# petuum/autodist

Measured on AMD Instinct MI355X. Metric: images/sec ResNet-50 AllReduce, higher is better.
Workload: dtype bf16; 1 GPU; model=resnet50, global_batch=512, parallelism=dp1, image_size=224

## Files before the change

### autodist_amd/models/resnet.py

```python
import torch
import torch.nn as nn


def _make_bn(ch, fused, relu):
    if fused:
        from autodist_amd.ops.fused_bn import FusedBatchNorm2d
        return FusedBatchNorm2d(ch, relu=relu)
    return nn.BatchNorm2d(ch)


class Bottleneck(nn.Module):
    expansion = 4

    def __init__(self, in_ch, width, stride=1, downsample=None, fused=False):
        super().__init__()
        out_ch = width * self.expansion
        self.fused = fused
        self.conv1 = nn.Conv2d(in_ch, width, 1, bias=False)
        self.bn1 = _make_bn(width, fused, relu=True)
        self.conv2 = nn.Conv2d(width, width, 3, stride=stride, padding=1,
                               bias=False)
        self.bn2 = _make_bn(width, fused, relu=True)
        self.conv3 = nn.Conv2d(width, out_ch, 1, bias=False)
        self.bn3 = _make_bn(out_ch, fused, relu=True)
        self.relu = nn.ReLU(inplace=True)
        self.downsample = downsample

    def forward(self, x):
        if self.fused:
            out = self.bn1(self.conv1(x))
            out = self.bn2(self.conv2(out))
            z = self.conv3(out)
            if self.downsample is None:
                return self.bn3.forward_add(z, x)
            return self.bn3.forward_add_bn(z, self.downsample[0](x),
                                           self.downsample[1])
        identity = x
        out = self.relu(self.bn1(self.conv1(x)))
        out = self.relu(self.bn2(self.conv2(out)))
        out = self.bn3(self.conv3(out))
        if self.downsample is not None:
            identity = self.downsample(x)
        return self.relu(out + identity)


class BasicBlock(nn.Module):
    expansion = 1

    def __init__(self, in_ch, width, stride=1, downsample=None, fused=False):
        super().__init__()
        self.fused = fused
        self.conv1 = nn.Conv2d(in_ch, width, 3, stride=stride, padding=1,
                               bias=False)
        self.bn1 = _make_bn(width, fused, relu=True)
        self.conv2 = nn.Conv2d(width, width, 3, padding=1, bias=False)
        self.bn2 = _make_bn(width, fused, relu=True)
        self.relu = nn.ReLU(inplace=True)
        self.downsample = downsample

    def forward(self, x):
        if self.fused:
            out = self.bn1(self.conv1(x))
            z = self.conv2(out)
            if self.downsample is None:
                return self.bn2.forward_add(z, x)
            return self.bn2.forward_add_bn(z, self.downsample[0](x),
                                           self.downsample[1])
        identity = x
        out = self.relu(self.bn1(self.conv1(x)))
        out = self.bn2(self.conv2(out))
        if self.downsample is not None:
            identity = self.downsample(x)
        return self.relu(out + identity)


class ResNet(nn.Module):
    def __init__(self, block, layers, num_classes=1000, fused=False):
        super().__init__()
        self.in_ch = 64
        self.fused = fused
        self.conv1 = nn.Conv2d(3, 64, 7, stride=2, padding=3, bias=False)
        self.bn1 = _make_bn(64, fused, relu=True)
        self.relu = nn.ReLU(inplace=True)
        self.maxpool = nn.MaxPool2d(3, stride=2, padding=1)
        self.layer1 = self._make_layer(block, 64, layers[0])
        self.layer2 = self._make_layer(block, 128, layers[1], stride=2)
        self.layer3 = self._make_layer(block, 256, layers[2], stride=2)
        self.layer4 = self._make_layer(block, 512, layers[3], stride=2)
        self.avgpool = nn.AdaptiveAvgPool2d(1)
        self.fc = nn.Linear(512 * block.expansion, num_classes)
        from autodist_amd.ops.fused_bn import FusedBatchNorm2d
        for m in self.modules():
            if isinstance(m, nn.Conv2d):
                nn.init.kaiming_normal_(m.weight, mode="fan_out",
                                        nonlinearity="relu")
            elif isinstance(m, (nn.BatchNorm2d, FusedBatchNorm2d)):
                nn.init.ones_(m.weight)
                nn.init.zeros_(m.bias)

    def _make_layer(self, block, width, blocks, stride=1):
        downsample = None
        out_ch = width * block.expansion
        if stride != 1 or self.in_ch != out_ch:
            downsample = nn.Sequential(
                nn.Conv2d(self.in_ch, out_ch, 1, stride=stride, bias=False),
                _make_bn(out_ch, self.fused, relu=False))
        layers = [block(self.in_ch, width, stride, downsample,
                        fused=self.fused)]
        self.in_ch = out_ch
        for _ in range(1, blocks):
            layers.append(block(self.in_ch, width, fused=self.fused))
        return nn.Sequential(*layers)

    def forward(self, x):
        if self.fused:
            x = self.bn1.forward_pool(self.conv1(x))
        else:
            x = self.maxpool(self.relu(self.bn1(self.conv1(x))))
        x = self.layer4(self.layer3(self.layer2(self.layer1(x))))
        x = self.avgpool(x).flatten(1)
        return self.fc(x)


def resnet18(num_classes=1000, fused=False):
    return ResNet(BasicBlock, [2, 2, 2, 2], num_classes, fused=fused)


def resnet50(num_classes=1000, fused=False):
    return ResNet(Bottleneck, [3, 4, 6, 3], num_classes, fused=fused)


def resnet101(num_classes=1000, fused=False):
    return ResNet(Bottleneck, [3, 4, 23, 3], num_classes, fused=fused)
```

### autodist_amd/ops/csrc/bn_ops.hip

```cpp
#include "common.h"

#define BN_VEC 8
#define BN_RED_U 4
#define BN_FIN_U 8
#define BN_RELU_NONE 0
#define BN_RELU_Y 1
#define BN_RELU_MASK 2

__device__ __forceinline__ void load8(const __hip_bfloat16* p, float* v) {
  const __hip_bfloat162* p2 = reinterpret_cast<const __hip_bfloat162*>(p);
  float2 a = __bfloat1622float2(p2[0]);
  float2 b = __bfloat1622float2(p2[1]);
  float2 c = __bfloat1622float2(p2[2]);
  float2 d = __bfloat1622float2(p2[3]);
  v[0] = a.x; v[1] = a.y; v[2] = b.x; v[3] = b.y;
  v[4] = c.x; v[5] = c.y; v[6] = d.x; v[7] = d.y;
}
__device__ __forceinline__ void store8(__hip_bfloat16* p, const float* v) {
  __hip_bfloat162* p2 = reinterpret_cast<__hip_bfloat162*>(p);
  p2[0] = __float22bfloat162_rn({v[0], v[1]});
  p2[1] = __float22bfloat162_rn({v[2], v[3]});
  p2[2] = __float22bfloat162_rn({v[4], v[5]});
  p2[3] = __float22bfloat162_rn({v[6], v[7]});
}
// ... 390 lines not shown
  load8(dy + m * C + c0, dv);
  if (RELU == BN_RELU_Y) {
    float yv[BN_VEC];
    load8(y + m * C + c0, yv);
#pragma unroll
    for (int k = 0; k < BN_VEC; ++k) dv[k] = yv[k] > 0.f ? dv[k] : 0.f;
  }
  if (RELU == BN_RELU_MASK)
    apply_mask8(mask[m * (C / BN_VEC) + c0 / BN_VEC], dv);
}

template <typename T, int RELU>
__global__ void __launch_bounds__(BLOCK_THREADS)
__attribute__((amdgpu_waves_per_eu(RELU == BN_RELU_POOL ? 2 : 1)))
bn_bwd_reduce_kernel(const T* __restrict__ x, const T* __restrict__ dy,
                     const T* __restrict__ y,
                     const unsigned char* __restrict__ mask,
                     const float* __restrict__ save_mean,
                     const float* __restrict__ save_rstd,
                     float* __restrict__ partial_dz,
                     float* __restrict__ partial_dzxh, long M, int C,
                     BNPool pool) {
#pragma clang fp contract(off)
  int tx_count = min(C / BN_VEC, (int)blockDim.x);
  int tx = threadIdx.x % tx_count;
  int ty = threadIdx.x / tx_count;
  int rows_per_blk = blockDim.x / tx_count;
  int c0 = (blockIdx.y * tx_count + tx) * BN_VEC;
  if (c0 >= C) return;
  float mean[BN_VEC], rstd[BN_VEC];
  load8(save_mean + c0, mean);
  load8(save_rstd + c0, rstd);
  float s[BN_VEC] = {0}, t[BN_VEC] = {0};
  const long stride = (long)gridDim.x * rows_per_blk;
  long m = (long)blockIdx.x * rows_per_blk + ty;
  for (; m + (BN_RED_U - 1) * stride < M; m += BN_RED_U * stride) {
    Raw8<T> rx[BN_RED_U], rd[BN_RED_U], ry[BN_RED_U];
    unsigned rm[BN_RED_U];
    PoolTaps<T> rp[BN_RED_U];
#pragma unroll
    for (int u = 0; u < BN_RED_U; ++u) {
      const long mu = m + u * stride;
      rx[u] = load8raw(x + mu * C + c0);
      if (RELU == BN_RELU_POOL) {
        pool_issue(dy, pool, mu, C, c0, rp[u]);
        __builtin_amdgcn_sched_barrier(0);
      } else {
        rd[u] = load8raw(dy + mu * C + c0);
      }
      if (RELU == BN_RELU_Y) ry[u] = load8raw(y + mu * C + c0);
      if (RELU == BN_RELU_MASK) rm[u] = mask[mu * (C / BN_VEC) + c0 / BN_VEC];
    }
    __builtin_amdgcn_sched_barrier(0);
#pragma unroll
    for (int u = 0; u < BN_RED_U; ++u) {
      float xv[BN_VEC], dv[BN_VEC];
      unpack8(rx[u], xv);
      if (RELU == BN_RELU_POOL) pool_dz(rp[u], dv);
      else unpack8(rd[u], dv);
      if (RELU == BN_RELU_Y) {
        float yv[BN_VEC];
        unpack8(ry[u], yv);
#pragma unroll
        for (int k = 0; k < BN_VEC; ++k) dv[k] = yv[k] > 0.f ? dv[k] : 0.f;
      }
      if (RELU == BN_RELU_MASK) apply_mask8(rm[u], dv);
#pragma unroll
      for (int k = 0; k < BN_VEC; ++k) {
        s[k] += dv[k];
        t[k] = fmaf(dv[k] * (xv[k] - mean[k]), rstd[k], t[k]);
      }
      if (RELU == BN_RELU_POOL) __builtin_amdgcn_sched_barrier(0);
    }
  }
  for (; m < M; m += stride) {
    float xv[BN_VEC], dv[BN_VEC];
    load8(x + m * C + c0, xv);
    bn_load_dz<T, RELU>(dy, y, mask, pool, m, C, c0, dv);
#pragma unroll
    for (int k = 0; k < BN_VEC; ++k) {
      s[k] += dv[k];
      t[k] = fmaf(dv[k] * (xv[k] - mean[k]), rstd[k], t[k]);
    }
  }
  __shared__ float ls[BLOCK_THREADS * BN_VEC];
  __shared__ float lt[BLOCK_THREADS * BN_VEC];
#pragma unroll
  for (int k = 0; k < BN_VEC; ++k) {
    ls[threadIdx.x * BN_VEC + k] = s[k];
    lt[threadIdx.x * BN_VEC + k] = t[k];
  }
  __syncthreads();
  if (ty == 0) {
    for (int r = 1; r < rows_per_blk; ++r) {
      int o = (r * tx_count + tx) * BN_VEC;
#pragma unroll
      for (int k = 0; k < BN_VEC; ++k) { s[k] += ls[o + k]; t[k] += lt[o + k]; }
    }
    store8(partial_dz + (long)blockIdx.x * C + c0, s);
    store8(partial_dzxh + (long)blockIdx.x * C + c0, t);
  }
}

__global__ void bn_bwd_finalize_kernel(const float* __restrict__ partial_dz,
                                       const float* __restrict__ partial_dzxh,
                                       int grid_m,
                                       const float* __restrict__ weight,
                                       const float* __restrict__ save_rstd,
                                       float* __restrict__ k1,
                                       float* __restrict__ k2,
                                       float* __restrict__ k3,
                                       float* __restrict__ dweight,
                                       float* __restrict__ dbias, long M,
                                       int C) {
  int tx = threadIdx.x % FIN_CH;
  int ty = threadIdx.x / FIN_CH;
  int c = blockIdx.x * FIN_CH + tx;
  if (c >= C) return;
  float sdz = 0.f, sdzxh = 0.f;
  bn_fin_lane_sum(partial_dz, partial_dzxh, grid_m, ty, C, c, sdz, sdzxh);
  __shared__ float ls[FIN_LANES * FIN_CH], lq[FIN_LANES * FIN_CH];
  ls[ty * FIN_CH + tx] = sdz;
  lq[ty * FIN_CH + tx] = sdzxh;
  __syncthreads();
  if (ty != 0) return;
#pragma unroll
  for (int r = 1; r < FIN_LANES; ++r) {
    sdz += ls[r * FIN_CH + tx];
    sdzxh += lq[r * FIN_CH + tx];
  }
  k1[c] = weight[c] * save_rstd[c];
  k2[c] = sdz / (float)M;
  k3[c] = sdzxh / (float)M;
  dweight[c] = sdzxh;
  dbias[c] = sdz;
}

template <typename T, int RELU, bool ADD>
__global__ void bn_bwd_apply_kernel(const T* __restrict__ x,
                                    const T* __restrict__ dy,
                                    const T* __restrict__ y,
                                    const unsigned char* __restrict__ mask,
                                    const float* __restrict__ save_mean,
                                    const float* __restrict__ save_rstd,
                                    const float* __restrict__ k1,
                                    const float* __restrict__ k2,
                                    const float* __restrict__ k3,
                                    T* __restrict__ dx, T* __restrict__ dres,
                                    long M, int C, BNPool pool) {
  int tx_count = min(C / BN_VEC, (int)blockDim.x);
  int tx = threadIdx.x % tx_count;
  int ty = threadIdx.x / tx_count;
  int rows_per_blk = blockDim.x / tx_count;
  int c0 = (blockIdx.y * tx_count + tx) * BN_VEC;
  if (c0 >= C) return;
  float mean[BN_VEC], rstd[BN_VEC], a1[BN_VEC], a2[BN_VEC], a3[BN_VEC];
  load8(save_mean + c0, mean);
  load8(save_rstd + c0, rstd);
  load8(k1 + c0, a1);
  load8(k2 + c0, a2);
  load8(k3 + c0, a3);
  for (long m = (long)blockIdx.x * rows_per_blk + ty; m < M;
       m += (long)gridDim.x * rows_per_blk) {
    float xv[BN_VEC], dv[BN_VEC];
    load8(x + m * C + c0, xv);
    bn_load_dz<T, RELU>(dy, y, mask, pool, m, C, c0, dv);
// ... 11 lines not shown
```

### autodist_amd/ops/csrc/ext.hip

```cpp
#include <torch/extension.h>
#include <ATen/cuda/CUDAContext.h>

#include "multi_tensor.hip"
#include "bn_ops.hip"
#include "psgd_gemm.hip"
#include "mfma_probe.hip"
#include "attention.hip"
#include "attention_bwd.hip"
#include "ln_ops.hip"
#include "ce_ops.hip"

namespace {

inline hipStream_t cur_stream() {
  return at::cuda::getCurrentCUDAStream().stream();
}

struct BNGeom {
  long M;
  int C;
  int tx_count, rows_per_blk, grid_c;
};

BNGeom bn_geom(const torch::Tensor& x) {
// ... 289 lines not shown
  } else {
    yp = bn_ptr<const T>(yq);
  }
  float* wp = w5.data_ptr<float>();
  float* partial_dz = wp;
  float* partial_dzxh = wp + (long)BN_GM_MAX * g.C;
  float* k1 = wp + (long)(2 * BN_GM_MAX + 0) * g.C;
  float* k2 = wp + (long)(2 * BN_GM_MAX + 1) * g.C;
  float* k3 = wp + (long)(2 * BN_GM_MAX + 2) * g.C;
  auto dweight = torch::empty({g.C}, fopt);
  auto dbias = torch::empty({g.C}, fopt);
  auto dx = torch::empty_like(x);
  torch::Tensor dres;
  if (need_dres) dres = torch::empty_like(x);
  dim3 block(BLOCK_THREADS);
  int gm = bn_reduce_gm(g);
  dim3 grid_r(gm, g.grid_c);
  dim3 grid_a(bn_grid_m(g, 4096), g.grid_c);
  auto st = cur_stream();
  const float* sm = save_mean.data_ptr<float>();
  const float* sr = save_rstd.data_ptr<float>();

  hipLaunchKernelGGL((bn_bwd_reduce_kernel<T, RELU>), grid_r, block, 0, st,
                     bn_ptr<const T>(x), bn_ptr<const T>(dy), yp, mp, sm, sr,
                     partial_dz, partial_dzxh, g.M, g.C, BNPool{});
  hipLaunchKernelGGL(bn_bwd_finalize_kernel,
                     dim3((g.C + FIN_CH - 1) / FIN_CH),
                     dim3(FIN_CH * FIN_LANES), 0, st, partial_dz,
                     partial_dzxh, gm, weight.data_ptr<float>(), sr, k1, k2,
                     k3, dweight.data_ptr<float>(), dbias.data_ptr<float>(),
                     g.M, g.C);
  if (need_dres)
    hipLaunchKernelGGL((bn_bwd_apply_kernel<T, RELU, true>), grid_a, block, 0,
                       st, bn_ptr<const T>(x), bn_ptr<const T>(dy), yp, mp,
                       sm, sr, k1, k2, k3, bn_ptr<T>(dx), bn_ptr<T>(dres),
                       g.M, g.C, BNPool{});
  else
    hipLaunchKernelGGL((bn_bwd_apply_kernel<T, RELU, false>), grid_a, block,
                       0, st, bn_ptr<const T>(x), bn_ptr<const T>(dy), yp, mp,
                       sm, sr, k1, k2, k3, bn_ptr<T>(dx), (T*)nullptr, g.M,
                       g.C, BNPool{});
  std::vector<torch::Tensor> out = {dx, dweight, dbias};
  if (need_dres) out.push_back(dres);
  return out;
}

template <int RELU>
std::vector<torch::Tensor> bn_bwd_dispatch(
    const torch::Tensor& x, const torch::Tensor& dy, const torch::Tensor& yq,
    const torch::Tensor& save_mean, const torch::Tensor& save_rstd,
    const torch::Tensor& weight, bool need_dres,
    const c10::optional<torch::Tensor>& ws) {
  if (x.scalar_type() == torch::kBFloat16)
    return bn_bwd_impl<__hip_bfloat16, RELU>(x, dy, yq, save_mean, save_rstd,
                                             weight, need_dres, ws);
  TORCH_CHECK(x.scalar_type() == torch::kFloat32);
  return bn_bwd_impl<float, RELU>(x, dy, yq, save_mean, save_rstd, weight,
                                  need_dres, ws);
}

std::vector<torch::Tensor> bn_bwd(torch::Tensor x, torch::Tensor dy,
                                  torch::Tensor y, torch::Tensor save_mean,
                                  torch::Tensor save_rstd,
                                  torch::Tensor weight, bool relu,
                                  bool need_dres,
                                  c10::optional<torch::Tensor> ws) {
  if (relu)
    return bn_bwd_dispatch<BN_RELU_Y>(x, dy, y, save_mean, save_rstd, weight,
                                      need_dres, ws);
  return bn_bwd_dispatch<BN_RELU_NONE>(x, dy, y, save_mean, save_rstd, weight,
                                       need_dres, ws);
}

std::vector<torch::Tensor> bn_bwd_mask(torch::Tensor x, torch::Tensor dy,
                                       torch::Tensor mask,
                                       torch::Tensor save_mean,
                                       torch::Tensor save_rstd,
                                       torch::Tensor weight, bool relu,
                                       bool need_dres,
                                       c10::optional<torch::Tensor> ws) {
  TORCH_CHECK(relu, "the mask is the ReLU mask: relu must be set");
  return bn_bwd_dispatch<BN_RELU_MASK>(x, dy, mask, save_mean, save_rstd,
                                       weight, need_dres, ws);
}

template <typename T>
std::vector<torch::Tensor> bn_bwd_pool_impl(
    const torch::Tensor& x, const torch::Tensor& dy,
    const torch::Tensor& argmax, const torch::Tensor& save_mean,
    const torch::Tensor& save_rstd, const torch::Tensor& weight,
    const c10::optional<torch::Tensor>& ws) {
  auto g = bn_geom(x);
  BNPool p = bn_pool_geom(x, g);
  const long Mo = x.size(0) * (long)p.Ho * p.Wo;
  TORCH_CHECK(dy.dim() == 4 && dy.size(0) == x.size(0) && dy.size(1) == g.C &&
                  dy.size(2) == p.Ho && dy.size(3) == p.Wo &&
                  dy.scalar_type() == x.scalar_type() &&
                  dy.device() == x.device() &&
                  dy.is_contiguous(at::MemoryFormat::ChannelsLast),
              "dy must be the channels_last [N, C, Ho, Wo] gradient of the "
              "pooled y");
  TORCH_CHECK(argmax.scalar_type() == torch::kInt32 && argmax.is_contiguous() &&
                  argmax.dim() == 2 && argmax.size(0) == Mo &&
                  argmax.size(1) == g.C / BN_VEC &&
                  argmax.device() == x.device(),
              "argmax must be the [N*Ho*Wo, C/8] int32 tensor of "
              "bn_fwd_train_pool");
  p.amax = bn_ptr<const unsigned>(argmax);
  auto fopt = weight.options().dtype(torch::kFloat32);
  torch::Tensor w5 = ws.has_value() ? *ws
      : torch::empty({2 * BN_GM_MAX + 3, (long)g.C}, fopt);
  TORCH_CHECK(w5.size(0) >= 2 * BN_GM_MAX + 3 && w5.size(1) == g.C &&
              w5.is_contiguous());
  float* wp = w5.data_ptr<float>();
  float* partial_dz = wp;
  float* partial_dzxh = wp + (long)BN_GM_MAX * g.C;
  float* k1 = wp + (long)(2 * BN_GM_MAX + 0) * g.C;
  float* k2 = wp + (long)(2 * BN_GM_MAX + 1) * g.C;
  float* k3 = wp + (long)(2 * BN_GM_MAX + 2) * g.C;
  auto dweight = torch::empty({g.C}, fopt);
  auto dbias = torch::empty({g.C}, fopt);
  auto dx = torch::empty_like(x);
  dim3 block(BLOCK_THREADS);
  int gm = bn_reduce_gm(g);
  dim3 grid_r(gm, g.grid_c);
  dim3 grid_a(bn_grid_m(g, 4096), g.grid_c);
  auto st = cur_stream();
  const float* sm = save_mean.data_ptr<float>();
  const float* sr = save_rstd.data_ptr<float>();
  hipLaunchKernelGGL((bn_bwd_reduce_kernel<T, BN_RELU_POOL>), grid_r, block, 0,
                     st, bn_ptr<const T>(x), bn_ptr<const T>(dy),
                     (const T*)nullptr, (const unsigned char*)nullptr, sm, sr,
                     partial_dz, partial_dzxh, g.M, g.C, p);
  hipLaunchKernelGGL(bn_bwd_finalize_kernel,
                     dim3((g.C + FIN_CH - 1) / FIN_CH),
                     dim3(FIN_CH * FIN_LANES), 0, st, partial_dz,
                     partial_dzxh, gm, weight.data_ptr<float>(), sr, k1, k2,
                     k3, dweight.data_ptr<float>(), dbias.data_ptr<float>(),
                     g.M, g.C);
  hipLaunchKernelGGL((bn_bwd_apply_kernel<T, BN_RELU_POOL, false>), grid_a,
                     block, 0, st, bn_ptr<const T>(x), bn_ptr<const T>(dy),
                     (const T*)nullptr, (const unsigned char*)nullptr, sm, sr,
                     k1, k2, k3, bn_ptr<T>(dx), (T*)nullptr, g.M, g.C, p);
  return {dx, dweight, dbias};
}

std::vector<torch::Tensor> bn_bwd_pool(torch::Tensor x, torch::Tensor dy,
                                       torch::Tensor argmax,
                                       torch::Tensor save_mean,
                                       torch::Tensor save_rstd,
                                       torch::Tensor weight,
                                       c10::optional<torch::Tensor> ws) {
  if (x.scalar_type() == torch::kBFloat16)
    return bn_bwd_pool_impl<__hip_bfloat16>(x, dy, argmax, save_mean,
                                            save_rstd, weight, ws);
  TORCH_CHECK(x.scalar_type() == torch::kFloat32);
  return bn_bwd_pool_impl<float>(x, dy, argmax, save_mean, save_rstd, weight,
                                 ws);
}

void check_f32_flat(const torch::Tensor& t, const char* name) {
  TORCH_CHECK(t.is_cuda(), name, " must be on GPU");
  TORCH_CHECK(t.is_contiguous(), name, " must be contiguous");
  TORCH_CHECK(t.scalar_type() == torch::kFloat32, name, " must be fp32");
}

// ... 595 lines not shown
  long N = logits.size(0), H = logits.size(1);
  auto fopt = logits.options().dtype(torch::kFloat32);
  auto loss_rows = torch::empty({N}, fopt);
  auto m = torch::empty({N}, fopt);
  auto l2s = torch::empty({N}, fopt);
  hipLaunchKernelGGL(ce_fwd_kernel, dim3(N), dim3(256), 0, cur_stream(),
                     reinterpret_cast<__hip_bfloat16*>(logits.data_ptr()),
                     targets.data_ptr<long>(), loss_rows.data_ptr<float>(),
                     m.data_ptr<float>(), l2s.data_ptr<float>(), N, H);
  return {loss_rows, m, l2s};
}

torch::Tensor ce_bwd(torch::Tensor logits, torch::Tensor targets,
                     torch::Tensor m, torch::Tensor l2s,
                     torch::Tensor dloss_rows) {
  long N = logits.size(0), H = logits.size(1);
  auto dlogits = torch::empty_like(logits);
  hipLaunchKernelGGL(ce_bwd_kernel, dim3(N), dim3(256), 0, cur_stream(),
                     reinterpret_cast<__hip_bfloat16*>(logits.data_ptr()),
                     targets.data_ptr<long>(), m.data_ptr<float>(),
                     l2s.data_ptr<float>(),
                     dloss_rows.contiguous().data_ptr<float>(),
                     reinterpret_cast<__hip_bfloat16*>(dlogits.data_ptr()),
                     N, H);
  return dlogits;
}

torch::Tensor mfma_probe(torch::Tensor A, torch::Tensor B, long cand) {
  TORCH_CHECK(A.scalar_type() == torch::kBFloat16 && A.numel() == 16 * 32);
  TORCH_CHECK(B.scalar_type() == torch::kBFloat16 && B.numel() == 32 * 16);
  auto D = torch::zeros({16, 16}, A.options().dtype(torch::kFloat32));
  hipLaunchKernelGGL(mfma_probe_kernel, dim3(1), dim3(64), 0, cur_stream(),
                     reinterpret_cast<__hip_bfloat16*>(A.data_ptr()),
                     reinterpret_cast<__hip_bfloat16*>(B.data_ptr()),
                     D.data_ptr<float>(), (int)cand);
  return D;
}

void psgd_add_err_pad(torch::Tensor flat, torch::Tensor err,
                      torch::Tensor out) {
  long numel = flat.numel();
  long total = out.numel();
  hipLaunchKernelGGL(psgd_add_err_pad_kernel, dim3(grid_for(total, 1)),
                     dim3(BLOCK_THREADS), 0, cur_stream(),
                     flat.data_ptr<float>(), err.data_ptr<float>(),
                     out.data_ptr<float>(), numel, total);
}

}

PYBIND11_MODULE(TORCH_EXTENSION_NAME, m) {
  m.def("fused_sgd", &fused_sgd, "fused flat SGD update (gfx950)");
  m.def("fused_adam", &fused_adam, "fused flat Adam/AdamW update (gfx950)");
  m.def("fused_adagrad", &fused_adagrad,
        "fused flat Adagrad update (gfx950)");
  m.def("fused_sgd_wire", &fused_sgd_wire,
        "fused flat SGD update, bf16 wire gradient (gfx950)");
  m.def("fused_adam_wire", &fused_adam_wire,
        "fused flat Adam/AdamW update, bf16 wire gradient (gfx950)");
  m.def("fused_adagrad_wire", &fused_adagrad_wire,
        "fused flat Adagrad update, bf16 wire gradient (gfx950)");
  m.def("fused_rmsprop", &fused_rmsprop,
        "fused flat RMSprop update (gfx950, centered/momentum variants)");
  m.def("scale_cast_bf16", &scale_cast_bf16, "scale+cast fp32->bf16");
  m.def("cast_back_f32", &cast_back_f32, "cast bf16->fp32");
  m.def("ef_compress", &ef_compress, "fused error-feedback bf16 compress");
  m.def("segment_coalesce", &segment_coalesce,
        "dedup-sum row-sparse gradient");
  m.def("scatter_add_rows", &scatter_add_rows, "rowwise scatter-add");
  m.def("gather_rows", &gather_rows, "rowwise gather");
  m.def("sparse_apply_rows", &sparse_apply_rows,
        "fused row-wise SGD/Adagrad/Adam update of unique rows (gfx950)");
  m.def("bn_fwd_train", &bn_fwd_train,
        "fused NHWC batchnorm fwd (+add+relu), returns y/save_mean/save_rstd");
  m.def("bn_bwd", &bn_bwd,
        "fused NHWC batchnorm bwd (+relu-mask+dres), returns "
        "dx/dweight/dbias[/dres]");
  m.def("bn_fwd_train_mask", &bn_fwd_train_mask,
        "bn_fwd_train with relu that also returns the bit-packed ReLU mask "
        "[M, C/8] uint8");
  m.def("bn_bwd_mask", &bn_bwd_mask,
        "bn_bwd that takes the packed mask of bn_fwd_train_mask in place of "
        "y");
  m.def("bn_fwd_train_pool", &bn_fwd_train_pool,
        "bn + relu + 3x3/stride 2/pad 1 max-pool: (x, weight, bias, "
        "running_mean, running_var, eps, momentum, ws) -> (pooled y, "
        "save_mean, save_rstd, argmax words)");
  m.def("bn_bwd_pool", &bn_bwd_pool,
        "backward of bn_fwd_train_pool: (x, dy_pooled, argmax, save_mean, "
        "save_rstd, weight, ws) -> (dx, dweight, dbias)");
  m.def("bn_fwd_train_add_bn", &bn_fwd_train_add_bn,
        "relu(bn(z) + bn_d(zd)): (z, zd, then weight, bias, running_mean, "
        "running_var, eps, momentum, ws of each BN) -> (y, mask, save_mean, "
        "save_rstd, save_mean_d, save_rstd_d)");
  m.attr("BN_RED_U") = BN_RED_U;
  m.attr("BN_FIN_U") = BN_FIN_U;
  m.def("psgd_mq", &psgd_mq, "PowerSGD P = M @ Q (MFMA f32 16x16x4)");
  m.def("psgd_mtp", &psgd_mtp, "PowerSGD Qn = M^T @ P (MFMA f32 16x16x4)");
  m.def("psgd_decompress_ef", &psgd_decompress_ef,
        "fused hat = P Q^T * scale; err = M - hat; flat = hat");
  m.def("psgd_add_err_pad", &psgd_add_err_pad,
        "padded M = flat + err (zero tail)");
  m.def("mfma_probe", &mfma_probe,
        "diagnostic: v_mfma_f32_16x16x32_bf16 A/B layout probe");
  m.def("ce_fwd", &ce_fwd,
        "fused online-softmax cross-entropy fwd -> loss_rows, m, l2s");
  m.def("ce_bwd", &ce_bwd, "fused cross-entropy bwd -> dlogits (bf16)");
  m.def("col_sum", &col_sum, "bf16 [N,H] column sum -> fp32 [H]");
  m.def("ln_fwd", &ln_fwd,
        "fused bf16 LayerNorm(+residual) forward -> y, u, mean, rstd");
  m.def("ln_bwd", &ln_bwd, "fused bf16 LayerNorm backward -> dx, dgamma, "
        "dbeta");
  m.def("attn_dropmask", &attn_dropmask,
        "materialize the hash dropout keep-mask (testing)");
  m.def("attn_fwd", &attn_fwd,
        "fused MFMA attention forward (bf16, D=64; optional additive key "
        "mask + hash dropout) — 4-wave LDS-tiled",
        py::arg("q"), py::arg("k"), py::arg("v"), py::arg("scale"),
        py::arg("mask") = py::none(), py::arg("p_drop") = 0.0,
        py::arg("seed") = 0);
  m.def("attn_bwd", &attn_bwd,
        "fused MFMA attention backward (GPU-validated) -> dq, dk, dv",
        py::arg("q"), py::arg("k"), py::arg("v"), py::arg("o"),
        py::arg("dout"), py::arg("scale"), py::arg("mask") = py::none(),
        py::arg("p_drop") = 0.0, py::arg("seed") = 0);
}
```

### autodist_amd/ops/fused_bn.py

```python
from typing import Optional

import torch

from autodist_amd.ops import api as ops_api


SPLIT_PATH = False


class _FusedBNFunction(torch.autograd.Function):
    @staticmethod
    def forward(ctx, x, weight, bias, running_mean, running_var,
                momentum, eps, relu, residual, ws=None):
        use_hip = x.is_cuda and ops_api.has_gpu_ops()
        ctx.ws_bwd = ws[1] if ws is not None else None
        if use_hip and relu:
            y, save_mean, save_rstd, sign = ops_api.ext().bn_fwd_train_mask(
                x, weight, bias, running_mean, running_var, residual,
                eps, momentum, relu, ws[0] if ws is not None else None)
        elif use_hip:
            y, save_mean, save_rstd = ops_api.ext().bn_fwd_train(
                x, weight, bias, running_mean, running_var, residual,
                eps, momentum, relu, ws[0] if ws is not None else None)
            sign = y
        else:
            xf = x.float()
            m = xf.numel() // xf.size(1)
            with torch.no_grad():
                if m > 1:
                    y, save_mean, save_rstd = torch.native_batch_norm(
                        xf, weight, bias, running_mean, running_var, True,
                        momentum, eps)
                else:
                    y, save_mean, save_rstd = torch.native_batch_norm(
                        xf, weight, bias, None, None, True, momentum, eps)
                    running_mean.mul_(1 - momentum).add_(save_mean,
                                                         alpha=momentum)
                    running_var.mul_(1 - momentum)
                if residual is not None:
                    y = y + residual.float()
                if relu:
                    y = torch.relu(y)
                y = y.to(x.dtype)
            sign = y
        ctx.save_for_backward(x, sign, save_mean, save_rstd, weight)
        ctx.relu = relu
        ctx.has_res = residual is not None
        return y

    @staticmethod
    def backward(ctx, dy):
        x, sign, save_mean, save_rstd, weight = ctx.saved_tensors
        relu, has_res = ctx.relu, ctx.has_res
        use_hip = x.is_cuda and ops_api.has_gpu_ops()
        if use_hip:
            bwd = ops_api.ext().bn_bwd_mask if relu else ops_api.ext().bn_bwd
            out = bwd(x, dy.contiguous(
                memory_format=torch.channels_last), sign, save_mean, save_rstd,
                weight, relu, has_res, ctx.ws_bwd)
            dx, dweight, dbias = out[0], out[1], out[2]
            dres = out[3] if has_res else None
        else:
            dyf = dy.float()
            if relu:
                dyf = dyf * (sign > 0).float()
            dres = dyf.to(dy.dtype) if has_res else None
            dxf, dweight, dbias = torch.ops.aten.native_batch_norm_backward(
                dyf, x.float(), weight, None, None, save_mean, save_rstd,
                True, 0.0, [True, True, True])
            dx = dxf.to(x.dtype)
        return (dx, dweight, dbias, None, None, None, None, None, dres, None)


class _FusedBNPoolFunction(torch.autograd.Function):

    @staticmethod
    def forward(ctx, x, weight, bias, running_mean, running_var, momentum,
                eps, ws):
        y, save_mean, save_rstd, argmax = ops_api.ext().bn_fwd_train_pool(
            x, weight, bias, running_mean, running_var, eps, momentum,
            ws[0] if ws is not None else None)
        ctx.ws_bwd = ws[1] if ws is not None else None
        ctx.save_for_backward(x, argmax, save_mean, save_rstd, weight)
        return y

    @staticmethod
    def backward(ctx, dy):
        x, argmax, save_mean, save_rstd, weight = ctx.saved_tensors
        dx, dweight, dbias = ops_api.ext().bn_bwd_pool(
            x, dy.contiguous(memory_format=torch.channels_last), argmax,
            save_mean, save_rstd, weight, ctx.ws_bwd)
        return dx, dweight, dbias, None, None, None, None, None


class _FusedBNAddBNFunction(torch.autograd.Function):

    @staticmethod
    def forward(ctx, z, zd, weight, bias, running_mean, running_var, momentum,
                eps, ws, weight_d, bias_d, running_mean_d, running_var_d,
                momentum_d, eps_d, ws_d):
        y, mask, sm, sr, sm_d, sr_d = ops_api.ext().bn_fwd_train_add_bn(
            z, zd, weight, bias, running_mean, running_var, eps, momentum,
            ws[0] if ws is not None else None,
            weight_d, bias_d, running_mean_d, running_var_d, eps_d,
            momentum_d, ws_d[0] if ws_d is not None else None)
        ctx.ws_bwd = ws[1] if ws is not None else None
        ctx.ws_bwd_d = ws_d[1] if ws_d is not None else None
        ctx.save_for_backward(z, zd, mask, sm, sr, sm_d, sr_d, weight,
                              weight_d)
        return y

    @staticmethod
    def backward(ctx, dy):
        z, zd, mask, sm, sr, sm_d, sr_d, weight, weight_d = ctx.saved_tensors
        dy = dy.contiguous(memory_format=torch.channels_last)
        bwd = ops_api.ext().bn_bwd_mask
        dz, dw, db = bwd(z, dy, mask, sm, sr, weight, True, False, ctx.ws_bwd)
        dzd, dw_d, db_d = bwd(zd, dy, mask, sm_d, sr_d, weight_d, True, False,
                              ctx.ws_bwd_d)
        return (dz, dzd, dw, db, None, None, None, None, None,
                dw_d, db_d, None, None, None, None, None)


def fused_bn_train(x, weight, bias, running_mean, running_var,
                   momentum=0.1, eps=1e-5, relu=False,
                   residual: Optional[torch.Tensor] = None, ws=None):
    return _FusedBNFunction.apply(x, weight, bias, running_mean, running_var,
                                  momentum, eps, relu, residual, ws)


class FusedBatchNorm2d(torch.nn.Module):

    def __init__(self, num_features, eps=1e-5, momentum=0.1, relu=False):
        super().__init__()
        self.num_features = num_features
        self.eps = eps
        self.momentum = momentum
        self.relu = relu
        self.weight = torch.nn.Parameter(torch.ones(num_features))
        self.bias = torch.nn.Parameter(torch.zeros(num_features))
        self.register_buffer("running_mean", torch.zeros(num_features))
        self.register_buffer("running_var", torch.ones(num_features))
        self.register_buffer("num_batches_tracked",
                             torch.tensor(0, dtype=torch.long))
        self._ws = None

    def _check(self, x):
        if x.is_cuda and not x.is_contiguous(memory_format=torch.channels_last):
            x = x.contiguous(memory_format=torch.channels_last)
        return x

    def _workspace(self, x):
        if not x.is_cuda:
            return None
        if self._ws is None or self._ws[0].device != x.device:
            self._ws = (
                torch.empty(2 * 512 + 4, self.num_features, device=x.device),
                torch.empty(2 * 512 + 3, self.num_features, device=x.device))
        return self._ws

    def forward(self, x, residual: Optional[torch.Tensor] = None):
        x = self._check(x)
        if residual is not None:
            residual = self._check(residual)
        if self.training:
            self.num_batches_tracked += 1
            return fused_bn_train(x, self.weight, self.bias,
                                  self.running_mean, self.running_var,
                                  self.momentum, self.eps, self.relu, residual,
                                  ws=self._workspace(x))
        scale = self.weight * (self.running_var + self.eps).rsqrt()
        shift = self.bias - self.running_mean * scale
        y = x * scale[None, :, None, None].to(x.dtype) + \
            shift[None, :, None, None].to(x.dtype)
        if residual is not None:
            y = y + residual
        return torch.relu(y) if self.relu else y

    def forward_add(self, x, residual):
        return self.forward(x, residual)

    def _fused_kernels(self, x):
        return (self.training and x.is_cuda and ops_api.has_gpu_ops()
                and not SPLIT_PATH)

    def forward_pool(self, x):
        assert self.relu, "forward_pool is bn -> relu -> max-pool"
        if not self._fused_kernels(x):
            return torch.nn.functional.max_pool2d(self.forward(x), 3, 2, 1)
        x = self._check(x)
        self.num_batches_tracked += 1
        return _FusedBNPoolFunction.apply(
            x, self.weight, self.bias, self.running_mean, self.running_var,
            self.momentum, self.eps, self._workspace(x))

    def forward_add_bn(self, z, zd, other_bn):
        if not (self._fused_kernels(z) and self.relu
                and isinstance(other_bn, FusedBatchNorm2d)
                and other_bn.training and not other_bn.relu):
            return self.forward_add(z, other_bn(zd))
        z, zd = self._check(z), other_bn._check(zd)
        self.num_batches_tracked += 1
        other_bn.num_batches_tracked += 1
        return _FusedBNAddBNFunction.apply(
            z, zd, self.weight, self.bias, self.running_mean,
            self.running_var, self.momentum, self.eps, self._workspace(z),
            other_bn.weight, other_bn.bias, other_bn.running_mean,
            other_bn.running_var, other_bn.momentum, other_bn.eps,
            other_bn._workspace(zd))

    def extra_repr(self):
        return f"{self.num_features}, relu={self.relu}"
```

Before: 9638 images/sec.

## Fuse residual gradient add into BN backward reduce via paired block outputs

```diff
diff --git a/autodist_amd/models/resnet.py b/autodist_amd/models/resnet.py
--- a/autodist_amd/models/resnet.py
+++ b/autodist_amd/models/resnet.py
@@ -26,15 +26,19 @@
         self.relu = nn.ReLU(inplace=True)
         self.downsample = downsample
 
+    def forward_pair(self, xs):
+        x_main, x_res = xs
+        out = self.bn1(self.conv1(x_main))
+        out = self.bn2(self.conv2(out))
+        z = self.conv3(out)
+        if self.downsample is None:
+            return self.bn3.forward_add_pair(z, x_res)
+        return self.bn3.forward_add_bn_pair(z, self.downsample[0](x_res),
+                                            self.downsample[1])
+
     def forward(self, x):
         if self.fused:
-            out = self.bn1(self.conv1(x))
-            out = self.bn2(self.conv2(out))
-            z = self.conv3(out)
-            if self.downsample is None:
-                return self.bn3.forward_add(z, x)
-            return self.bn3.forward_add_bn(z, self.downsample[0](x),
-                                           self.downsample[1])
+            return self.forward_pair((x, x))[0]
         identity = x
         out = self.relu(self.bn1(self.conv1(x)))
         out = self.relu(self.bn2(self.conv2(out)))
@@ -58,14 +62,18 @@
         self.relu = nn.ReLU(inplace=True)
         self.downsample = downsample
 
+    def forward_pair(self, xs):
+        x_main, x_res = xs
+        out = self.bn1(self.conv1(x_main))
+        z = self.conv2(out)
+        if self.downsample is None:
+            return self.bn2.forward_add_pair(z, x_res)
+        return self.bn2.forward_add_bn_pair(z, self.downsample[0](x_res),
+                                            self.downsample[1])
+
     def forward(self, x):
         if self.fused:
-            out = self.bn1(self.conv1(x))
-            z = self.conv2(out)
-            if self.downsample is None:
-                return self.bn2.forward_add(z, x)
-            return self.bn2.forward_add_bn(z, self.downsample[0](x),
-                                           self.downsample[1])
+            return self.forward_pair((x, x))[0]
         identity = x
         out = self.relu(self.bn1(self.conv1(x)))
         out = self.bn2(self.conv2(out))
@@ -115,9 +123,14 @@
     def forward(self, x):
         if self.fused:
             x = self.bn1.forward_pool(self.conv1(x))
+            xs = (x, x)
+            for layer in (self.layer1, self.layer2, self.layer3, self.layer4):
+                for block in layer:
+                    xs = block.forward_pair(xs)
+            x = xs[0]
         else:
             x = self.maxpool(self.relu(self.bn1(self.conv1(x))))
-        x = self.layer4(self.layer3(self.layer2(self.layer1(x))))
+            x = self.layer4(self.layer3(self.layer2(self.layer1(x))))
         x = self.avgpool(x).flatten(1)
         return self.fc(x)
 
diff --git a/autodist_amd/ops/csrc/bn_ops.hip b/autodist_amd/ops/csrc/bn_ops.hip
--- a/autodist_amd/ops/csrc/bn_ops.hip
+++ b/autodist_amd/ops/csrc/bn_ops.hip
@@ -496,6 +496,102 @@
       s[k] += dv[k];
       t[k] = fmaf(dv[k] * (xv[k] - mean[k]), rstd[k], t[k]);
     }
+  }
+  __shared__ float ls[BLOCK_THREADS * BN_VEC];
+  __shared__ float lt[BLOCK_THREADS * BN_VEC];
+#pragma unroll
+  for (int k = 0; k < BN_VEC; ++k) {
+    ls[threadIdx.x * BN_VEC + k] = s[k];
+    lt[threadIdx.x * BN_VEC + k] = t[k];
+  }
+  __syncthreads();
+  if (ty == 0) {
+    for (int r = 1; r < rows_per_blk; ++r) {
+      int o = (r * tx_count + tx) * BN_VEC;
+#pragma unroll
+      for (int k = 0; k < BN_VEC; ++k) { s[k] += ls[o + k]; t[k] += lt[o + k]; }
+    }
+    store8(partial_dz + (long)blockIdx.x * C + c0, s);
+    store8(partial_dzxh + (long)blockIdx.x * C + c0, t);
+  }
+}
+
+#ifndef BN_JOIN_U
+#define BN_JOIN_U 4
+#endif
+template <typename T>
+__device__ __forceinline__ void bn_join_dz8(const float* av, const float* bv,
+                                            unsigned bits, float* dv) {
+#pragma clang fp contract(off)
+#pragma unroll
+  for (int k = 0; k < BN_VEC; ++k)
+    dv[k] = (bits >> k) & 1u ? round_to(av[k] + bv[k], (const T*)nullptr)
+                             : 0.f;
+}
+
+template <typename T>
+__global__ void __launch_bounds__(BLOCK_THREADS)
+__attribute__((amdgpu_waves_per_eu(1)))
+bn_bwd_reduce_join_kernel(const T* __restrict__ x, const T* __restrict__ dy_a,
+                          const T* __restrict__ dy_b,
+                          const unsigned char* __restrict__ mask,
+                          const float* __restrict__ save_mean,
+                          const float* __restrict__ save_rstd,
+                          float* __restrict__ partial_dz,
+                          float* __restrict__ partial_dzxh,
+                          T* __restrict__ dz, long M, int C) {
+#pragma clang fp contract(off)
+  int tx_count = min(C / BN_VEC, (int)blockDim.x);
+  int tx = threadIdx.x % tx_count;
+  int ty = threadIdx.x / tx_count;
+  int rows_per_blk = blockDim.x / tx_count;
+  int c0 = (blockIdx.y * tx_count + tx) * BN_VEC;
+  if (c0 >= C) return;
+  float mean[BN_VEC], rstd[BN_VEC];
+  load8(save_mean + c0, mean);
+  load8(save_rstd + c0, rstd);
+  float s[BN_VEC] = {0}, t[BN_VEC] = {0};
+  const long stride = (long)gridDim.x * rows_per_blk;
+  long m = (long)blockIdx.x * rows_per_blk + ty;
+  for (; m + (BN_JOIN_U - 1) * stride < M; m += BN_JOIN_U * stride) {
+    Raw8<T> rx[BN_JOIN_U], ra[BN_JOIN_U], rb[BN_JOIN_U];
+    unsigned rm[BN_JOIN_U];
+#pragma unroll
+    for (int u = 0; u < BN_JOIN_U; ++u) {
+      const long mu = m + u * stride;
+      rx[u] = load8raw(x + mu * C + c0);
+      ra[u] = load8raw(dy_a + mu * C + c0);
+      rb[u] = load8raw(dy_b + mu * C + c0);
+      rm[u] = mask[mu * (C / BN_VEC) + c0 / BN_VEC];
+    }
+    __builtin_amdgcn_sched_barrier(0);
+#pragma unroll
+    for (int u = 0; u < BN_JOIN_U; ++u) {
+      float xv[BN_VEC], av[BN_VEC], bv[BN_VEC], dv[BN_VEC];
+      unpack8(rx[u], xv);
+      unpack8(ra[u], av);
+      unpack8(rb[u], bv);
+      bn_join_dz8<T>(av, bv, rm[u], dv);
+#pragma unroll
+      for (int k = 0; k < BN_VEC; ++k) {
+        s[k] += dv[k];
+        t[k] = fmaf(dv[k] * (xv[k] - mean[k]), rstd[k], t[k]);
+      }
+      store8(dz + (m + u * stride) * C + c0, dv);
+    }
+  }
+  for (; m < M; m += stride) {
+    float xv[BN_VEC], av[BN_VEC], bv[BN_VEC], dv[BN_VEC];
+    load8(x + m * C + c0, xv);
+    load8(dy_a + m * C + c0, av);
+    load8(dy_b + m * C + c0, bv);
+    bn_join_dz8<T>(av, bv, mask[m * (C / BN_VEC) + c0 / BN_VEC], dv);
+#pragma unroll
+    for (int k = 0; k < BN_VEC; ++k) {
+      s[k] += dv[k];
+      t[k] = fmaf(dv[k] * (xv[k] - mean[k]), rstd[k], t[k]);
+    }
+    store8(dz + m * C + c0, dv);
   }
   __shared__ float ls[BLOCK_THREADS * BN_VEC];
   __shared__ float lt[BLOCK_THREADS * BN_VEC];
diff --git a/autodist_amd/ops/csrc/ext.hip b/autodist_amd/ops/csrc/ext.hip
--- a/autodist_amd/ops/csrc/ext.hip
+++ b/autodist_amd/ops/csrc/ext.hip
@@ -395,6 +395,79 @@
   TORCH_CHECK(relu, "the mask is the ReLU mask: relu must be set");
   return bn_bwd_dispatch<BN_RELU_MASK>(x, dy, mask, save_mean, save_rstd,
                                        weight, need_dres, ws);
+}
+
+template <typename T>
+std::vector<torch::Tensor> bn_bwd_mask_join_impl(
+    const torch::Tensor& x, const torch::Tensor& dy_a,
+    const torch::Tensor& dy_b, const torch::Tensor& mask,
+    const torch::Tensor& save_mean, const torch::Tensor& save_rstd,
+    const torch::Tensor& weight, const c10::optional<torch::Tensor>& ws) {
+  auto g = bn_geom(x);
+  for (const torch::Tensor* d : {&dy_a, &dy_b})
+    TORCH_CHECK(d->sizes() == x.sizes() &&
+                    d->scalar_type() == x.scalar_type() &&
+                    d->device() == x.device() &&
+                    d->is_contiguous(at::MemoryFormat::ChannelsLast),
+                "bn_bwd_mask_join: dy_a and dy_b must match x in shape, "
+                "dtype, device and channels_last layout");
+  auto fopt = weight.options().dtype(torch::kFloat32);
+  torch::Tensor w5 = ws.has_value() ? *ws
+      : torch::empty({2 * BN_GM_MAX + 3, (long)g.C}, fopt);
+  TORCH_CHECK(w5.size(0) >= 2 * BN_GM_MAX + 3 && w5.size(1) == g.C &&
+              w5.is_contiguous());
+  TORCH_CHECK(mask.scalar_type() == torch::kUInt8 && mask.is_contiguous() &&
+                  mask.dim() == 2 && mask.size(0) == g.M &&
+                  mask.size(1) == g.C / BN_VEC && mask.device() == x.device(),
+              "mask must be the [M, C/8] uint8 tensor of bn_fwd_train_mask");
+  const unsigned char* mp = mask.data_ptr<unsigned char>();
+  float* wp = w5.data_ptr<float>();
+  float* partial_dz = wp;
+  float* partial_dzxh = wp + (long)BN_GM_MAX * g.C;
+  float* k1 = wp + (long)(2 * BN_GM_MAX + 0) * g.C;
+  float* k2 = wp + (long)(2 * BN_GM_MAX + 1) * g.C;
+  float* k3 = wp + (long)(2 * BN_GM_MAX + 2) * g.C;
+  auto dweight = torch::empty({g.C}, fopt);
+  auto dbias = torch::empty({g.C}, fopt);
+  auto dx = torch::empty_like(x);
+  auto dz = torch::empty_like(x);
+  dim3 block(BLOCK_THREADS);
+  int gm = bn_reduce_gm(g);
+  dim3 grid_r(gm, g.grid_c);
+  dim3 grid_a(bn_grid_m(g, 4096), g.grid_c);
+  auto st = cur_stream();
+  const float* sm = save_mean.data_ptr<float>();
+  const float* sr = save_rstd.data_ptr<float>();
+
+  hipLaunchKernelGGL((bn_bwd_reduce_join_kernel<T>), grid_r, block, 0, st,
+                     bn_ptr<const T>(x), bn_ptr<const T>(dy_a),
+                     bn_ptr<const T>(dy_b), mp, sm, sr, partial_dz,
+                     partial_dzxh, bn_ptr<T>(dz), g.M, g.C);
+  hipLaunchKernelGGL(bn_bwd_finalize_kernel,
+                     dim3((g.C + FIN_CH - 1) / FIN_CH),
+                     dim3(FIN_CH * FIN_LANES), 0, st, partial_dz,
+                     partial_dzxh, gm, weight.data_ptr<float>(), sr, k1, k2,
+                     k3, dweight.data_ptr<float>(), dbias.data_ptr<float>(),
+                     g.M, g.C);
+  hipLaunchKernelGGL((bn_bwd_apply_kernel<T, BN_RELU_NONE, false>), grid_a,
+                     block, 0, st, bn_ptr<const T>(x), bn_ptr<const T>(dz),
+                     (const T*)nullptr, (const unsigned char*)nullptr, sm, sr,
+                     k1, k2, k3, bn_ptr<T>(dx), (T*)nullptr, g.M, g.C,
+                     BNPool{});
+  return {dx, dweight, dbias, dz};
+}
+
+std::vector<torch::Tensor> bn_bwd_mask_join(
+    torch::Tensor x, torch::Tensor dy_a, torch::Tensor dy_b,
+    torch::Tensor mask, torch::Tensor save_mean, torch::Tensor save_rstd,
+    torch::Tensor weight, c10::optional<torch::Tensor> ws) {
+  if (x.scalar_type() == torch::kBFloat16)
+    return bn_bwd_mask_join_impl<__hip_bfloat16>(x, dy_a, dy_b, mask,
+                                                 save_mean, save_rstd, weight,
+                                                 ws);
+  TORCH_CHECK(x.scalar_type() == torch::kFloat32);
+  return bn_bwd_mask_join_impl<float>(x, dy_a, dy_b, mask, save_mean,
+                                      save_rstd, weight, ws);
 }
 
 template <typename T>
@@ -1156,6 +1229,10 @@
   m.def("bn_bwd_mask", &bn_bwd_mask,
         "bn_bwd that takes the packed mask of bn_fwd_train_mask in place of "
         "y");
+  m.def("bn_bwd_mask_join", &bn_bwd_mask_join,
+        "bn_bwd_mask for dy = dy_a + dy_b, the add done in the reduce: (x, "
+        "dy_a, dy_b, mask, save_mean, save_rstd, weight, ws) -> (dx, "
+        "dweight, dbias, dz); dz is the masked sum, the split path's dres");
   m.def("bn_fwd_train_pool", &bn_fwd_train_pool,
         "bn + relu + 3x3/stride 2/pad 1 max-pool: (x, weight, bias, "
         "running_mean, running_var, eps, momentum, ws) -> (pooled y, "
@@ -1169,6 +1246,7 @@
         "save_rstd, save_mean_d, save_rstd_d)");
   m.attr("BN_RED_U") = BN_RED_U;
   m.attr("BN_FIN_U") = BN_FIN_U;
+  m.attr("BN_JOIN_U") = BN_JOIN_U;
   m.def("psgd_mq", &psgd_mq, "PowerSGD P = M @ Q (MFMA f32 16x16x4)");
   m.def("psgd_mtp", &psgd_mtp, "PowerSGD Qn = M^T @ P (MFMA f32 16x16x4)");
   m.def("psgd_decompress_ef", &psgd_decompress_ef,
diff --git a/autodist_amd/ops/fused_bn.py b/autodist_amd/ops/fused_bn.py
--- a/autodist_amd/ops/fused_bn.py
+++ b/autodist_amd/ops/fused_bn.py
@@ -8,11 +8,22 @@
 SPLIT_PATH = False
 
 
+def _two_handles(ctx, y):
+    ctx.set_materialize_grads(False)
+    return y, y.view_as(y)
+
+
+def _nhwc_grad(g):
+    return None if g is None else g.contiguous(
+        memory_format=torch.channels_last)
+
+
 class _FusedBNFunction(torch.autograd.Function):
     @staticmethod
     def forward(ctx, x, weight, bias, running_mean, running_var,
-                momentum, eps, relu, residual, ws=None):
+                momentum, eps, relu, residual, ws=None, pair=False):
         use_hip = x.is_cuda and ops_api.has_gpu_ops()
+        assert not pair or (use_hip and relu and residual is not None)
         ctx.ws_bwd = ws[1] if ws is not None else None
         if use_hip and relu:
             y, save_mean, save_rstd, sign = ops_api.ext().bn_fwd_train_mask(
@@ -46,14 +57,22 @@
         ctx.save_for_backward(x, sign, save_mean, save_rstd, weight)
         ctx.relu = relu
         ctx.has_res = residual is not None
-        return y
-
-    @staticmethod
-    def backward(ctx, dy):
+        return _two_handles(ctx, y) if pair else y
+
+    @staticmethod
+    def backward(ctx, dy, dy_b=None):
         x, sign, save_mean, save_rstd, weight = ctx.saved_tensors
         relu, has_res = ctx.relu, ctx.has_res
         use_hip = x.is_cuda and ops_api.has_gpu_ops()
-        if use_hip:
+        if dy is None:
+            dy, dy_b = dy_b, None
+            if dy is None:
+                return (None,) * 11
+        if dy_b is not None:
+            dx, dweight, dbias, dres = ops_api.ext().bn_bwd_mask_join(
+                x, _nhwc_grad(dy), _nhwc_grad(dy_b), sign, save_mean,
+                save_rstd, weight, ctx.ws_bwd)
+        elif use_hip:
             bwd = ops_api.ext().bn_bwd_mask if relu else ops_api.ext().bn_bwd
             out = bwd(x, dy.contiguous(
                 memory_format=torch.channels_last), sign, save_mean, save_rstd,
@@ -69,7 +88,8 @@
                 dyf, x.float(), weight, None, None, save_mean, save_rstd,
                 True, 0.0, [True, True, True])
             dx = dxf.to(x.dtype)
-        return (dx, dweight, dbias, None, None, None, None, None, dres, None)
+        return (dx, dweight, dbias, None, None, None, None, None, dres, None,
+                None)
 
 
 class _FusedBNPoolFunction(torch.autograd.Function):
@@ -98,7 +118,7 @@
     @staticmethod
     def forward(ctx, z, zd, weight, bias, running_mean, running_var, momentum,
                 eps, ws, weight_d, bias_d, running_mean_d, running_var_d,
-                momentum_d, eps_d, ws_d):
+                momentum_d, eps_d, ws_d, pair=False):
         y, mask, sm, sr, sm_d, sr_d = ops_api.ext().bn_fwd_train_add_bn(
             z, zd, weight, bias, running_mean, running_var, eps, momentum,
             ws[0] if ws is not None else None,
@@ -108,25 +128,38 @@
         ctx.ws_bwd_d = ws_d[1] if ws_d is not None else None
         ctx.save_for_backward(z, zd, mask, sm, sr, sm_d, sr_d, weight,
                               weight_d)
-        return y
-
-    @staticmethod
-    def backward(ctx, dy):
+        return _two_handles(ctx, y) if pair else y
+
+    @staticmethod
+    def backward(ctx, dy, dy_b=None):
         z, zd, mask, sm, sr, sm_d, sr_d, weight, weight_d = ctx.saved_tensors
-        dy = dy.contiguous(memory_format=torch.channels_last)
-        bwd = ops_api.ext().bn_bwd_mask
-        dz, dw, db = bwd(z, dy, mask, sm, sr, weight, True, False, ctx.ws_bwd)
-        dzd, dw_d, db_d = bwd(zd, dy, mask, sm_d, sr_d, weight_d, True, False,
-                              ctx.ws_bwd_d)
+        if dy is None:
+            dy, dy_b = dy_b, None
+            if dy is None:
+                return (None,) * 17
+        dy = _nhwc_grad(dy)
+        if dy_b is not None:
+            dz, dw, db, dym = ops_api.ext().bn_bwd_mask_join(
+                z, dy, _nhwc_grad(dy_b), mask, sm, sr, weight, ctx.ws_bwd)
+            dzd, dw_d, db_d = ops_api.ext().bn_bwd(
+                zd, dym, dym, sm_d, sr_d, weight_d, False, False,
+                ctx.ws_bwd_d)
+        else:
+            bwd = ops_api.ext().bn_bwd_mask
+            dz, dw, db = bwd(z, dy, mask, sm, sr, weight, True, False,
+                             ctx.ws_bwd)
+            dzd, dw_d, db_d = bwd(zd, dy, mask, sm_d, sr_d, weight_d, True,
+                                  False, ctx.ws_bwd_d)
         return (dz, dzd, dw, db, None, None, None, None, None,
-                dw_d, db_d, None, None, None, None, None)
+                dw_d, db_d, None, None, None, None, None, None)
 
 
 def fused_bn_train(x, weight, bias, running_mean, running_var,
                    momentum=0.1, eps=1e-5, relu=False,
-                   residual: Optional[torch.Tensor] = None, ws=None):
+                   residual: Optional[torch.Tensor] = None, ws=None,
+                   pair=False):
     return _FusedBNFunction.apply(x, weight, bias, running_mean, running_var,
-                                  momentum, eps, relu, residual, ws)
+                                  momentum, eps, relu, residual, ws, pair)
 
 
 class FusedBatchNorm2d(torch.nn.Module):
@@ -184,6 +217,17 @@
         return (self.training and x.is_cuda and ops_api.has_gpu_ops()
                 and not SPLIT_PATH)
 
+    def forward_add_pair(self, x, residual):
+        if not (self._fused_kernels(x) and self.relu):
+            y = self.forward_add(x, residual)
+            return y, y
+        self.num_batches_tracked += 1
+        return fused_bn_train(self._check(x), self.weight, self.bias,
+                              self.running_mean, self.running_var,
+                              self.momentum, self.eps, True,
+                              self._check(residual), ws=self._workspace(x),
+                              pair=True)
+
     def forward_pool(self, x):
         assert self.relu, "forward_pool is bn -> relu -> max-pool"
         if not self._fused_kernels(x):
@@ -194,11 +238,15 @@
             x, self.weight, self.bias, self.running_mean, self.running_var,
             self.momentum, self.eps, self._workspace(x))
 
-    def forward_add_bn(self, z, zd, other_bn):
+    def forward_add_bn_pair(self, z, zd, other_bn):
+        return self.forward_add_bn(z, zd, other_bn, pair=True)
+
+    def forward_add_bn(self, z, zd, other_bn, pair=False):
         if not (self._fused_kernels(z) and self.relu
                 and isinstance(other_bn, FusedBatchNorm2d)
                 and other_bn.training and not other_bn.relu):
-            return self.forward_add(z, other_bn(zd))
+            y = self.forward_add(z, other_bn(zd))
+            return (y, y) if pair else y
         z, zd = self._check(z), other_bn._check(zd)
         self.num_batches_tracked += 1
         other_bn.num_batches_tracked += 1
@@ -207,7 +255,7 @@
             self.running_var, self.momentum, self.eps, self._workspace(z),
             other_bn.weight, other_bn.bias, other_bn.running_mean,
             other_bn.running_var, other_bn.momentum, other_bn.eps,
-            other_bn._workspace(zd))
+            other_bn._workspace(zd), pair)
 
     def extra_repr(self):
         return f"{self.num_features}, relu={self.relu}"
```

New measurement: 9996 images/sec, median of 6. +3.7%, better.
